# helmholtz-analytics/mpi4torch

Measured on AMD Instinct MI355X. Metric: allreduce_fwdbwd_algbw_GBps, higher is better.
Workload: dtype bf16; 1 GPU; model=allreduce_1GiB_bf16_fwd_bwd, parallelism=dp1

## Files before the change

### csrc/extension.cpp

```cpp

#include "ops.hpp"
#include "transport.hpp"

#include <torch/script.h>
#include <torch/extension.h>

#include <rccl/rccl.h>

namespace m4a {
namespace {

std::string& world_group_name() {
  static std::string name;
  return name;
}

c10::intrusive_ptr<Communicator> comm_world() {
  return c10::make_intrusive<Communicator>(world_group_name());
}

c10::intrusive_ptr<Communicator> comm_from_group(std::string group_name) {
  return c10::make_intrusive<Communicator>(std::move(group_name));
}

// ... 54 lines not shown

  m.def("_set_world_group_name",
        [](const std::string& name) { m4a::world_group_name() = name; });
  m.def("_get_world_group_name",
        []() { return m4a::world_group_name(); });

  m.def("force_host_staging",
        [](bool enabled) { m4a::config().force_host_staging = enabled; });
  m.def("host_staging_forced",
        []() { return m4a::config().force_host_staging; });

  m.def("force_full_path",
        [](bool enabled) { m4a::config().force_full_path = enabled; });

  m.def("_pack_roundtrip", &m4a::debug_pack_roundtrip);
  m.def("_slab_copy", &m4a::debug_slab_copy);
  m.def("_unpack_blocks", &m4a::debug_unpack_blocks);
  m.def("_pack_blocks", &m4a::debug_pack_blocks);
  m.def("_bitwise_reduce", &m4a::debug_bitwise_reduce);
  m.def("_fp8_reduce", &m4a::debug_fp8_reduce);
  m.def("_arith_reduce", &m4a::debug_arith_reduce);
  m.def("_pairloc_reduce", &m4a::debug_pairloc_reduce);
  m.def("_mx8_quantize", &m4a::debug_mx8_quantize);
  m.def("_mx8_reduce", &m4a::debug_mx8_reduce);
  m.def("_mx8_dequantize", &m4a::debug_mx8_dequantize, py::arg("payload"),
        py::arg("scales"), py::arg("numel"), py::arg("dtype"),
        py::arg("out") = c10::optional<at::Tensor>());
  m.def("_mx8_reduce_to", &m4a::debug_mx8_reduce_to, py::arg("payload"),
        py::arg("scales"), py::arg("numel"), py::arg("dtype"),
        py::arg("out") = c10::optional<at::Tensor>());
  m.def("_mx8_dequantize_blocks", &m4a::debug_mx8_dequantize_blocks,
// ... 30 lines not shown
```

### csrc/kernels.hip

```cpp

#include <hip/hip_runtime.h>
#include <hip/hip_fp8.h>
#include "kernels.hpp"

namespace m4a {

namespace {

struct SlabArgs {
  const char* src;
  char* dst;
  long long row_b;
  long long chunks_per_row;
  long long total_chunks;
  long long src_pitch_b;
  long long dst_pitch_b;
};

template <int N>
struct SlabPack {
  SlabArgs s[N];
};

typedef unsigned int v4u __attribute__((ext_vector_type(4)));
template <typename T>
struct NtVec {
  using type = T;
};
template <>
struct NtVec<uint4> {
  using type = v4u;
};

template <typename VecT, int NSLABS>
__global__ __launch_bounds__(256) void slab_copy_kernel(SlabPack<NSLABS> pack) {
  constexpr long long G = (long long)sizeof(VecT);
  const SlabArgs& a = pack.s[blockIdx.z];
  const long long stride = (long long)gridDim.x * blockDim.x;
  for (long long i = (long long)blockIdx.x * blockDim.x + threadIdx.x;
       i < a.total_chunks; i += stride) {
    const long long b = i / a.chunks_per_row;
    const long long c = i - b * a.chunks_per_row;
    const char* srow = a.src + b * a.src_pitch_b;
    char* drow = a.dst + b * a.dst_pitch_b;
    long long head =
        (G - ((long long)(uintptr_t)drow & (G - 1))) & (G - 1);
    if (head > a.row_b) head = a.row_b;
    const long long body = (a.row_b - head) / G;
    if (c < body) {
      using NT = typename NtVec<VecT>::type;
      const NT* sp = reinterpret_cast<const NT*>(srow + head) + c;
      NT* dp = reinterpret_cast<NT*>(drow + head) + c;
      __builtin_nontemporal_store(__builtin_nontemporal_load(sp), dp);
    } else {
      for (long long k = 0; k < head; ++k) drow[k] = srow[k];
      for (long long k = head + body * G; k < a.row_b; ++k) drow[k] = srow[k];
    }
  }
}

template <typename VecT>
void launch_bucket(const SlabDesc* descs, int n, hipStream_t stream) {
  constexpr long long G = (long long)sizeof(VecT);
  while (n > 0) {
    const int take = n < kMaxSlabsPerLaunch ? n : kMaxSlabsPerLaunch;
    SlabPack<kMaxSlabsPerLaunch> pack{};
    long long max_chunks = 0;
    for (int i = 0; i < take; ++i) {
      const SlabDesc& d = descs[i];
      SlabArgs& a = pack.s[i];
      a.src = static_cast<const char*>(d.src);
      a.dst = static_cast<char*>(d.dst);
      a.row_b = d.count * d.after_b;
      a.src_pitch_b = d.src_pitch_b;
      a.dst_pitch_b = d.dst_pitch_b;
      a.chunks_per_row = (a.row_b >= G ? a.row_b / G : 0) + 1;
      a.total_chunks = d.before * a.chunks_per_row;
      if (a.total_chunks > max_chunks) max_chunks = a.total_chunks;
    }
    for (int i = take; i < kMaxSlabsPerLaunch; ++i) {
      pack.s[i] = pack.s[0];
      pack.s[i].total_chunks = 0;
    }
    if (max_chunks > 0) {
      long long blocks = (max_chunks + 255) / 256;
      if (blocks > 4096) blocks = 4096;
      if (blocks < 1) blocks = 1;
      dim3 grid((unsigned)blocks, 1, (unsigned)take);
      hipLaunchKernelGGL((slab_copy_kernel<VecT, kMaxSlabsPerLaunch>), grid,
                         dim3(256), 0, stream, pack);
    }
    descs += take;
    n -= take;
  }
}


template <int Q>
__device__ inline uint4 byte_window_q(const unsigned int d[8], int rbits) {
  if (rbits == 0) return make_uint4(d[Q], d[Q + 1], d[Q + 2], d[Q + 3]);
  auto take = [&](int j) {
    unsigned long long w =
        ((unsigned long long)d[Q + j + 1] << 32) | d[Q + j];
    return (unsigned int)(w >> rbits);
  };
  return make_uint4(take(0), take(1), take(2), take(3));
}

__device__ inline uint4 byte_window(const uint4& lo, const uint4& hi, int s) {
  const unsigned int d[8] = {lo.x, lo.y, lo.z, lo.w, hi.x, hi.y, hi.z, hi.w};
  const int q = s >> 2;
  const int rbits = (s & 3) * 8;
  switch (q) {
    case 0: return byte_window_q<0>(d, rbits);
    case 1: return byte_window_q<1>(d, rbits);
    case 2: return byte_window_q<2>(d, rbits);
    default: return byte_window_q<3>(d, rbits);
  }
}

template <int NSLABS>
__global__ __launch_bounds__(256) void slab_copy_shift_kernel(
    SlabPack<NSLABS> pack) {
  const SlabArgs& a = pack.s[blockIdx.z];
  const long long stride = (long long)gridDim.x * blockDim.x;
  for (long long i = (long long)blockIdx.x * blockDim.x + threadIdx.x;
       i < a.total_chunks; i += stride) {
    const long long b = i / a.chunks_per_row;
    const long long c = i - b * a.chunks_per_row;
    const char* srow = a.src + b * a.src_pitch_b;
    char* drow = a.dst + b * a.dst_pitch_b;
    long long head = (16 - ((long long)(uintptr_t)drow & 15)) & 15;
    if (head > a.row_b) head = a.row_b;
    const long long body = (a.row_b - head) / 16;
    const char* sbase = srow + head;
    const int s = (int)((uintptr_t)sbase & 15);
    const long long bodyv = (s == 0) ? body : (body > 0 ? body - 1 : 0);
    const long long vs = (s == 0 || s <= head) ? 0 : 1;
    if (c >= vs && c < bodyv) {
      const char* sal = sbase - s + 16 * c;
      if (s == 0) {
        __builtin_nontemporal_store(
            __builtin_nontemporal_load(reinterpret_cast<const v4u*>(sal)),
            reinterpret_cast<v4u*>(drow + head + 16 * c));
      } else {
        const uint4 lo = *reinterpret_cast<const uint4*>(sal);
        const uint4 hi = *reinterpret_cast<const uint4*>(sal + 16);
        const uint4 w = byte_window(lo, hi, s);
        __builtin_nontemporal_store(
            *reinterpret_cast<const v4u*>(&w),
            reinterpret_cast<v4u*>(drow + head + 16 * c));
      }
    } else if (c == bodyv) {
      if (bodyv <= vs) {
        for (long long k = 0; k < a.row_b; ++k) drow[k] = srow[k];
      } else {
        const long long lo_end = head + vs * 16;
        for (long long k = 0; k < lo_end; ++k) drow[k] = srow[k];
        for (long long k = head + bodyv * 16; k < a.row_b; ++k) {
          drow[k] = srow[k];
        }
      }
    }
  }
}

void launch_shift_bucket(const SlabDesc* descs, int n, hipStream_t stream) {
  while (n > 0) {
    const int take = n < kMaxSlabsPerLaunch ? n : kMaxSlabsPerLaunch;
    SlabPack<kMaxSlabsPerLaunch> pack{};
    long long max_chunks = 0;
    for (int i = 0; i < take; ++i) {
      const SlabDesc& d = descs[i];
      SlabArgs& a = pack.s[i];
      a.src = static_cast<const char*>(d.src);
      a.dst = static_cast<char*>(d.dst);
      a.row_b = d.count * d.after_b;
      a.src_pitch_b = d.src_pitch_b;
      a.dst_pitch_b = d.dst_pitch_b;
      a.chunks_per_row = (a.row_b >= 16 ? a.row_b / 16 : 0) + 1;
      a.total_chunks = d.before * a.chunks_per_row;
      if (a.total_chunks > max_chunks) max_chunks = a.total_chunks;
    }
    for (int i = take; i < kMaxSlabsPerLaunch; ++i) {
      pack.s[i] = pack.s[0];
      pack.s[i].total_chunks = 0;
    }
    if (max_chunks > 0) {
      long long blocks = (max_chunks + 255) / 256;
      if (blocks > 4096) blocks = 4096;
      if (blocks < 1) blocks = 1;
      dim3 grid((unsigned)blocks, 1, (unsigned)take);
      hipLaunchKernelGGL((slab_copy_shift_kernel<kMaxSlabsPerLaunch>), grid,
                         dim3(256), 0, stream, pack);
    }
    descs += take;
    n -= take;
  }
}

inline int slab_granule(const SlabDesc& d) {
  const long long delta =
      (long long)((uintptr_t)d.src - (uintptr_t)d.dst);
  const long long pdelta = d.src_pitch_b - d.dst_pitch_b;
  for (int g = 16; g > 1; g >>= 1) {
    if ((delta & (g - 1)) == 0 && (pdelta & (g - 1)) == 0) return g;
  }
  return 1;
}
// ... 45 lines not shown

template <typename T, typename Op>
void launch_bitred(const void* in, void* out, int64_t chunk_elems, int nranks,
                   hipStream_t stream) {
  long long blocks = (chunk_elems + 255) / 256;
  if (blocks > 4096) blocks = 4096;
  if (blocks < 1) blocks = 1;
  hipLaunchKernelGGL((bitwise_reduce_kernel<T, Op>), dim3((unsigned)blocks),
                     dim3(256), 0, stream, static_cast<const T*>(in),
                     static_cast<T*>(out), (long long)chunk_elems,
                     (long long)nranks);
}

}

void launch_slab_copy(const SlabDesc* descs, int n, hipStream_t stream) {
  int i = 0;
  while (i < n) {
    const int g = slab_granule(descs[i]);
    int j = i + 1;
    while (j < n && slab_granule(descs[j]) == g) ++j;
    switch (g) {
      case 16: launch_bucket<uint4>(descs + i, j - i, stream); break;
      case 8: launch_bucket<unsigned long long>(descs + i, j - i, stream); break;
      case 4: launch_bucket<unsigned int>(descs + i, j - i, stream); break;
      default:
        launch_shift_bucket(descs + i, j - i, stream);
        break;
    }
    i = j;
  }
}

void launch_bitwise_reduce(const void* in, void* out, int64_t chunk_bytes,
                           int nranks, int op, hipStream_t stream) {
  const bool vec16 = (chunk_bytes % 16 == 0) &&
                     (reinterpret_cast<uintptr_t>(in) % 16 == 0) &&
                     (reinterpret_cast<uintptr_t>(out) % 16 == 0);
  if (vec16) {
    const int64_t elems = chunk_bytes / 16;
    switch (op) {
      case 0: launch_bitred<uint4, OpAnd>(in, out, elems, nranks, stream); break;
// ... 147 lines not shown
      launch_fp8_reduce_t<Op, true>(in, out, n_elems, nranks, stream);
    } else {
      launch_fp8_reduce_t<Op, false>(in, out, n_elems, nranks, stream);
    }
  };
  switch (op) {
    case 0: dispatch(FAdd{}); break;
    case 1: dispatch(FMul{}); break;
    case 2: dispatch(FMinNan{}); break;
    default: dispatch(FMaxNan{}); break;
  }
}


namespace {

constexpr long long kMaxGrid = 1ll << 30;

struct TF32 {
  using S = float;
  static constexpr int E = 4;
  __device__ static void unpack(v4u w, float* f) {
    for (int d = 0; d < 4; ++d) f[d] = __uint_as_float(w[d]);
  }
  __device__ static v4u pack(const float* f) {
    v4u o;
    for (int d = 0; d < 4; ++d) o[d] = __float_as_uint(f[d]);
    return o;
  }
  __device__ static float ld(const S* p) { return *p; }
  __device__ static void st(S* p, float f) { *p = f; }
};
// ... 122 lines not shown
    const char* __restrict__ src, char* __restrict__ dst, long long nvec,
    long long nbytes) {
  const long long items = nvec + (nbytes > nvec * 16 ? 1 : 0);
  for (long long t = blockIdx.x; t * 256 < items; t += gridDim.x) {
    const long long i = t * 256 + threadIdx.x;
    if (i < nvec) {
      __builtin_nontemporal_store(
          __builtin_nontemporal_load(reinterpret_cast<const v4u*>(src) + i),
          reinterpret_cast<v4u*>(dst) + i);
    } else if (i == nvec) {
      for (long long k = nvec * 16; k < nbytes; ++k) dst[k] = src[k];
    }
  }
}

inline unsigned arith_grid(long long items) {
  long long blocks = (items + 255) / 256;
  if (blocks > kMaxGrid) blocks = kMaxGrid;
  if (blocks < 1) blocks = 1;
  return (unsigned)blocks;
}

template <typename T, typename Op>
void launch_arith_reduce_t(const void* own, const void* staged,
                           int64_t stride_elems, int nranks, int me,
                           void* out, int64_t n, hipStream_t stream) {
  const long long esize = (long long)sizeof(typename T::S);
  const long long stride_b = (long long)stride_elems * esize;
  auto al16 = [](const void* p) {
    return reinterpret_cast<uintptr_t>(p) % 16 == 0;
  };
  const bool vec = al16(own) && al16(out) && al16(staged) && stride_b % 16 == 0;
  if (vec) {
    const long long nvec = n / T::E;
    const long long items = nvec + (n % T::E ? 1 : 0);
    hipLaunchKernelGGL((arith_reduce_kernel<T, Op>), dim3(arith_grid(items)),
                       dim3(256), 0, stream, static_cast<const char*>(own),
                       static_cast<const char*>(staged), stride_b, nranks, me,
                       static_cast<char*>(out), nvec, (long long)n);
  } else {
    hipLaunchKernelGGL((arith_reduce_kernel_scalar<T, Op>),
                       dim3(arith_grid(n)), dim3(256), 0, stream,
                       static_cast<const char*>(own),
                       static_cast<const char*>(staged), stride_b, nranks, me,
                       static_cast<char*>(out), (long long)n);
  }
}

}

void launch_arith_copy(const void* src, void* dst, int64_t nbytes,
                       hipStream_t stream) {
  if (nbytes <= 0) return;
  if (reinterpret_cast<uintptr_t>(src) % 16 != 0 ||
      reinterpret_cast<uintptr_t>(dst) % 16 != 0) {
    SlabDesc d;
    d.src = src;
    d.dst = dst;
    d.before = 1;
    d.count = 1;
    d.after_b = nbytes;
    d.src_pitch_b = nbytes;
    d.dst_pitch_b = nbytes;
    launch_slab_copy(&d, 1, stream);
    return;
  }
  const long long nvec = nbytes / 16;
  const long long items = nvec + (nbytes % 16 ? 1 : 0);
  hipLaunchKernelGGL(arith_reduce_copy_kernel, dim3(arith_grid(items)),
                     dim3(256), 0, stream, static_cast<const char*>(src),
                     static_cast<char*>(dst), nvec, (long long)nbytes);
}

void launch_arith_reduce(const void* own, const void* staged,
                         int64_t stride_elems, int nranks, int me, void* out,
                         int64_t n_elems, int op, int dtype,
                         hipStream_t stream) {
  if (n_elems <= 0) return;
  if (nranks == 1) {
    launch_arith_copy(own, out, n_elems * (dtype == 0 ? 4 : 2), stream);
    return;
  }
  auto dispatch = [&](auto opv) {
    using Op = decltype(opv);
    switch (dtype) {
      case 0:
// ... 124 lines not shown
```

### csrc/kernels.hpp

```cpp
#pragma once

#include <hip/hip_runtime_api.h>
#include <cstdint>

namespace m4a {

struct SlabDesc {
  const void* src;
  void* dst;
  int64_t before;
  int64_t count;
  int64_t after_b;
  int64_t src_pitch_b;
  int64_t dst_pitch_b;
};

constexpr int kMaxSlabsPerLaunch = 8;

void launch_slab_copy(const SlabDesc* descs, int n, hipStream_t stream);

void launch_bitwise_reduce(const void* in, void* out, int64_t chunk_bytes,
                           int nranks, int op, hipStream_t stream);

void launch_pairloc_reduce(const void* in, void* out, int64_t n_pairs,
                           int nranks, int op, int dtype, hipStream_t stream);

void launch_fp8_reduce(const void* in, void* out, int64_t n_elems,
                       int nranks, int op, bool e5m2, hipStream_t stream);

void launch_arith_reduce(const void* own, const void* staged,
                         int64_t stride_elems, int nranks, int me, void* out,
                         int64_t n_elems, int op, int dtype,
                         hipStream_t stream);
void launch_arith_copy(const void* src, void* dst, int64_t nbytes,
                       hipStream_t stream);

void launch_mx8_quantize(const void* in, void* payload, void* scales,
                         int64_t n_elems, int dtype, hipStream_t stream);
void launch_mx8_reduce(const void* payload_in, const void* scales_in,
                       void* payload_out, void* scales_out, int64_t n_groups,
                       int nranks, hipStream_t stream);
void launch_mx8_dequantize(const void* payload, const void* scales, void* out,
                           int64_t n_elems, int dtype, hipStream_t stream);
void launch_mx8_reduce_to(const void* payload_in, const void* scales_in,
                          void* out, int64_t n_elems, int nranks, int dtype,
                          hipStream_t stream);
void launch_mx8_dequantize_blocks(const void* payload, const void* scales,
                                  void* out, int nblocks, int64_t rows,
                                  int64_t row_elems, int dtype,
                                  hipStream_t stream);
// ... 6 lines not shown
```

### csrc/ops.cpp

```cpp

#include "ops.hpp"
#include "transport.hpp"
#include "kernels.hpp"

#include <torch/csrc/autograd/function.h>
#include <torch/csrc/autograd/functions/utils.h>
#include <torch/csrc/autograd/variable.h>
#include <ATen/core/TensorBody.h>
#include <ATen/WrapDimUtils.h>

#include <ATen/hip/impl/HIPStreamMasqueradingAsCUDA.h>

#include <algorithm>
#include <cstdlib>
#include <cstring>
#include <functional>
#include <limits>
#include <map>
#include <mutex>
#include <tuple>

namespace m4a {

using at::Tensor;
// ... 124 lines not shown
      auto b3 = blocks[i].view({g.before, counts[i], g.after})
                    .narrow(0, row_lo, rows);
      if (pack) {
        b3.copy_(f3.narrow(1, displs[i], counts[i]));
      } else {
        f3.narrow(1, displs[i], counts[i]).copy_(b3);
      }
    }
  }
}


Tensor fast_clone(const Tensor& in) {
  if (!in.is_cuda() || in.numel() == 0) return in.clone();
  auto out = at::empty_like(in);
  SlabDesc d;
  d.src = in.data_ptr();
  d.dst = out.data_ptr();
  d.before = 1;
  d.count = 1;
  d.after_b = in.numel() * in.element_size();
  d.src_pitch_b = d.after_b;
  d.dst_pitch_b = d.after_b;
  launch_slab_copy(&d, 1, current_gpu_stream(in));
  return out;
}

std::vector<int64_t> prefix_displs(const std::vector<int64_t>& counts) {
  std::vector<int64_t> d(counts.size(), 0);
  for (size_t i = 1; i < counts.size(); ++i) d[i] = d[i - 1] + counts[i - 1];
  return d;
}

int64_t phase_count(const Tensor& t, int64_t per_rank_bytes) {
  const int64_t c = config().pipeline_chunk_bytes;
  if (c <= 0) return 1;
  if (t.is_cuda()) {
    hipStreamCaptureStatus st = hipStreamCaptureStatusNone;
    (void)hipStreamIsCapturing(current_gpu_stream(t), &st);
// ... 2440 lines not shown
              "debug_pack_blocks expects a contiguous in [rows, P, row_elems] "
              "and flat staging [P*rows*row_elems] of the same dtype and "
              "device");
  const int64_t rows = in.size(0), P = in.size(1), re = in.size(2);
  if (in.numel() == 0) return;
  auto full = in.view({rows, P * re});
  std::vector<int64_t> counts((size_t)P, re);
  auto displs = prefix_displs(counts);
  std::vector<Tensor> blocks((size_t)P);
  for (int64_t r = 0; r < P; ++r) {
    blocks[(size_t)r] = staging.narrow(0, r * rows * re, rows * re);
  }
  move_axis_blocks(full, 1, displs, counts, blocks, true);
}

void debug_slab_copy(const Tensor& src, const Tensor& dst,
                     const std::vector<std::vector<int64_t>>& descs) {
  TORCH_CHECK(src.is_cuda() && dst.is_cuda() && src.device() == dst.device(),
              "debug_slab_copy is a GPU kernel test");
  TORCH_CHECK(src.scalar_type() == at::kByte && dst.scalar_type() == at::kByte &&
                  src.dim() == 1 && dst.dim() == 1 && src.is_contiguous() &&
                  dst.is_contiguous(),
              "debug_slab_copy expects flat contiguous uint8 tensors");
  constexpr int64_t kMaxBytes = int64_t(1) << 31;
  TORCH_CHECK(src.numel() < kMaxBytes && dst.numel() < kMaxBytes);
  const char* sbase = static_cast<const char*>(src.data_ptr());
  char* dbase = static_cast<char*>(dst.data_ptr());
  TORCH_CHECK(sbase + src.numel() <= dbase || dbase + dst.numel() <= sbase,
              "debug_slab_copy: src and dst overlap");
  auto span = [](int64_t off, int64_t before, int64_t row_b, int64_t pitch,
                 int64_t numel, size_t i, const char* side) {
    TORCH_CHECK(off >= 0 && off <= numel && before >= 0 && before <= numel &&
                    row_b >= 0 && row_b <= numel && pitch >= 0 &&
                    pitch <= numel,
                "debug_slab_copy: descriptor ", i, " out of range on ", side);
    if (before == 0 || row_b == 0) return std::make_pair(off, off);
    const int64_t end = off + (before - 1) * pitch + row_b;
    TORCH_CHECK(end <= numel, "debug_slab_copy: descriptor ", i,
                " runs past the end of ", side);
    return std::make_pair(off, end);
  };
  std::vector<SlabDesc> slabs;
  std::vector<std::pair<int64_t, int64_t>> dspans;
  slabs.reserve(descs.size());
// ... 17 lines not shown
    s.dst = dbase + t[1];
    s.before = before;
    s.count = count;
    s.after_b = after_b;
    s.src_pitch_b = t[5];
    s.dst_pitch_b = t[6];
    slabs.push_back(s);
  }
  std::sort(dspans.begin(), dspans.end());
  for (size_t i = 1; i < dspans.size(); ++i) {
    TORCH_CHECK(dspans[i - 1].second <= dspans[i].first,
                "debug_slab_copy: destination ranges overlap");
  }
  TORCH_CHECK(slabs.size() < (size_t)std::numeric_limits<int>::max());
  if (slabs.empty()) return;
  launch_slab_copy(slabs.data(), (int)slabs.size(), current_gpu_stream(src));
}

Tensor debug_fp8_reduce(const Tensor& stacked, int64_t op) {
  TORCH_CHECK(stacked.is_cuda(), "debug_fp8_reduce is a GPU kernel test");
  TORCH_CHECK(stacked.dim() >= 2);
  TORCH_CHECK(stacked.scalar_type() == at::kFloat8_e4m3fn ||
              stacked.scalar_type() == at::kFloat8_e5m2);
  auto in = stacked.contiguous();
  const int64_t n = in.size(0);
  auto out = at::empty(in.sizes().slice(1).vec(), in.options());
  launch_fp8_reduce(in.data_ptr(), out.data_ptr(), out.numel(), (int)n,
                    (int)op, in.scalar_type() == at::kFloat8_e5m2,
                    current_gpu_stream(in));
  return out;
}
// ... 222 lines not shown
```

### csrc/ops.hpp

```cpp
#pragma once

#include "common.hpp"

#include <ATen/ATen.h>
#include <torch/custom_class.h>

#include <memory>
#include <mutex>
#include <string>
#include <tuple>
#include <vector>

namespace m4a {

struct Transport;

struct Communicator : torch::CustomClassHolder {
  explicit Communicator(std::string group_name);

  int64_t GetRank();
  int64_t GetSize();

  at::Tensor Allreduce(const at::Tensor& input, int64_t op);
  at::Tensor AllreduceCompressed(const at::Tensor& input, int64_t op);
// ... 46 lines not shown

 private:
  std::string group_name_;
  std::mutex mu_;
  std::shared_ptr<Transport> cpu_tr_;
  std::shared_ptr<Transport> gpu_tr_;
  int gpu_device_ = -1;
};

at::Tensor join_dummies(const at::Tensor& loopthrough,
                        const std::vector<at::Tensor>& dummies);

at::Tensor debug_pack_roundtrip(const at::Tensor& input, int64_t axis,
                                std::vector<int64_t> counts);
void debug_slab_copy(const at::Tensor& src, const at::Tensor& dst,
                     const std::vector<std::vector<int64_t>>& descs);
at::Tensor debug_bitwise_reduce(const at::Tensor& stacked, int64_t op);
at::Tensor debug_fp8_reduce(const at::Tensor& stacked, int64_t op);
at::Tensor debug_arith_reduce(const at::Tensor& own, const at::Tensor& staged,
                              int64_t me, int64_t op);
std::tuple<at::Tensor, at::Tensor> debug_mx8_quantize(const at::Tensor& x);
std::tuple<at::Tensor, at::Tensor> debug_mx8_reduce(const at::Tensor& payload,
                                                    const at::Tensor& scales);
at::Tensor debug_mx8_dequantize(const at::Tensor& payload,
                                const at::Tensor& scales, int64_t numel,
                                at::ScalarType dtype,
                                const c10::optional<at::Tensor>& out);
at::Tensor debug_mx8_reduce_to(const at::Tensor& payload,
                               const at::Tensor& scales, int64_t numel,
                               at::ScalarType dtype,
                               const c10::optional<at::Tensor>& out);
// ... 15 lines not shown
```

### csrc/transport.cpp

```cpp

#include "transport.hpp"

#include <torch/csrc/distributed/c10d/Backend.hpp>
#include <torch/csrc/distributed/c10d/ProcessGroup.hpp>
#include <torch/csrc/distributed/c10d/GroupRegistry.hpp>
#include <torch/csrc/distributed/c10d/Types.hpp>

#include <ATen/hip/HIPContext.h>
#include <ATen/hip/impl/HIPStreamMasqueradingAsCUDA.h>
#include <ATen/hip/impl/HIPCachingAllocatorMasqueradingAsCUDA.h>
#include <ATen/hip/impl/HIPGuardImplMasqueradingAsCUDA.h>

#include <hip/hip_runtime_api.h>
#include <rccl/rccl.h>

#include <atomic>
#include <cstdlib>
#include <cstring>
#include <deque>
#include <map>
#include <mutex>
#include <unordered_map>

namespace m4a {
// ... 124 lines not shown
    return e;
  }
  void release(hipEvent_t e) {
    std::lock_guard<std::mutex> g(mu_);
    free_.push_back(e);
  }

 private:
  explicit EventPool(int dev) : dev_(dev) {}
  int dev_;
  std::mutex mu_;
  std::vector<hipEvent_t> free_;
};


struct SelfMatcher {
  struct Pending {
    uint64_t req_id;
    at::Tensor buf;
    int tag;
  };
  std::mutex mu;
  std::map<int, std::deque<Pending>> sends, recvs;

  static void check_tags(int stag, int rtag) {
    if (!config().debug_collectives) return;
    TORCH_CHECK(stag == rtag,
                "mpi4torch_amd[debug]: self send/recv matched FIFO but with "
                "different tags (send tag ", stag, ", recv tag ", rtag,
                "). Matching is FIFO per (peer, channel); tags do not "
                "reorder it — reorder your posts instead.");
  }

  static void complete_pair(const at::Tensor& src, at::Tensor& dst,
                            uint64_t sreq, uint64_t rreq) {
    dst.copy_(src, true);
    auto& tab = requests();
    std::lock_guard<std::mutex> g(tab.mu);
    for (uint64_t id : {sreq, rreq}) {
      Request* r = tab.peek(id);
      if (!r) continue;
      r->self_pending = false;
      if (src.is_cuda()) {
        r->gpu = true;
        r->device = (int)src.get_device();
        auto cur = c10::hip::getCurrentHIPStreamMasqueradingAsCUDA(r->device);
        r->event = EventPool::forDevice(r->device).acquire();
        M4A_HIP_CHECK(hipEventRecord(r->event, cur.stream()));
      }
    }
  }
// ... 144 lines not shown
      "disagrees: sender posted (tag=", m[0], ", dtype=",
      (at::ScalarType)m[1], ", numel=", m[2], ") but this rank's recv "
      "expected (tag=", r.debug_expect[0], ", dtype=",
      (at::ScalarType)r.debug_expect[1], ", numel=", r.debug_expect[2],
      "). Tags do not reorder matching; make both ranks post their "
      "transfers per peer+channel in the same order.");
}


struct LocalTransport final : Transport {
  int rank() const override { return 0; }
  int size() const override { return 1; }
  bool is_gpu() const override { return false; }

  void allreduce(const at::Tensor& in, at::Tensor& out, RedOp) override {
    out.copy_(in, true);
  }
  void broadcast(at::Tensor&, int) override {}
  void reduce(at::Tensor&, RedOp, int) override {}
  void allgather_equal(const at::Tensor& in, at::Tensor& out) override {
    out.view_as(in).copy_(in, true);
  }
  void reduce_scatter_equal(const at::Tensor& in, at::Tensor& out,
                            RedOp) override {
    out.copy_(in.view_as(out), true);
  }
  void exchange(const std::vector<at::Tensor>& sendbufs,
                const std::vector<int>& speers,
                std::vector<at::Tensor>& recvbufs,
                const std::vector<int>& rpeers) override {
    TORCH_CHECK(sendbufs.size() == recvbufs.size(),
                "local exchange requires matched self pairs");
    for (size_t i = 0; i < sendbufs.size(); ++i) {
      TORCH_CHECK(speers[i] == 0 && rpeers[i] == 0);
      recvbufs[i].view({-1}).copy_(sendbufs[i].reshape({-1}), true);
    }
  }
  uint64_t iexchange(const std::vector<at::Tensor>& sendbufs,
                     const std::vector<int>& speers,
                     std::vector<at::Tensor>& recvbufs,
                     const std::vector<int>& rpeers) override {
    exchange(sendbufs, speers, recvbufs, rpeers);
    Request r;
    r.buffers = recvbufs;
    if (!recvbufs.empty() && recvbufs[0].is_cuda()) {
      r.gpu = true;
      r.device = (int)recvbufs[0].get_device();
      auto cur = c10::hip::getCurrentHIPStreamMasqueradingAsCUDA(r.device);
      r.event = EventPool::forDevice(r.device).acquire();
      M4A_HIP_CHECK(hipEventRecord(r.event, cur.stream()));
// ... 7 lines not shown
  }
  uint64_t irecv(at::Tensor& buf, int peer, int tag, Channel ch) override {
    TORCH_CHECK(peer == 0, "world_size is 1; cannot receive from rank ", peer);
    return self_matcher().irecv(buf, tag, ch);
  }
  uint64_t ireduce_scatter(const at::Tensor& in, at::Tensor& out,
                           RedOp op) override {
    return iallreduce(in.view_as(out), out, op);
  }
  uint64_t iallgather(const at::Tensor& in, at::Tensor& out) override {
    auto v = out.view_as(in);
    return iallreduce(in, v, kSum);
  }
  uint64_t iallreduce(const at::Tensor& in, at::Tensor& out,
                      RedOp) override {
    out.copy_(in, true);
    Request r;
    r.buffer = out;
    if (out.is_cuda()) {
      r.gpu = true;
      r.device = (int)out.get_device();
      auto cur = c10::hip::getCurrentHIPStreamMasqueradingAsCUDA(r.device);
      r.event = EventPool::forDevice(r.device).acquire();
      M4A_HIP_CHECK(hipEventRecord(r.event, cur.stream()));
    }
    return requests().add(std::move(r));
  }
};


struct C10dTransport final : Transport {
// ... 282 lines not shown
    }
    for (size_t j = 0; j < recvbufs.size(); ++j) {
      if (rpeers[j] == me) {
        self_recvs.push_back(&recvbufs[j]);
        continue;
      }
      if (nbytes(recvbufs[j]) == 0) continue;
      M4A_NCCL_CHECK(ncclRecv(recvbufs[j].data_ptr(), nbytes(recvbufs[j]),
                              ncclUint8, rpeers[j], comm(Channel::Coll),
                              hop.stream()));
    }
    M4A_NCCL_CHECK(ncclGroupEnd());
    TORCH_CHECK(self_sends.size() == self_recvs.size(),
                "exchange: unmatched self blocks");
    for (size_t i = 0; i < self_sends.size(); ++i) {
      M4A_HIP_CHECK(hipMemcpyAsync(
          self_recvs[i]->data_ptr(), self_sends[i]->data_ptr(),
          nbytes(*self_sends[i]), hipMemcpyDeviceToDevice, hop.stream()));
    }
  }
  uint64_t isend(const at::Tensor& buf, int peer, int tag,
                 Channel ch) override {
    if (peer == rank_) return self_matcher().isend(buf, tag, ch);
    std::lock_guard<std::mutex> g(mu_);
    check_not_capturing("Isend");
    return defer_p2p(true, buf, peer, tag, ch);
  }
  uint64_t irecv(at::Tensor& buf, int peer, int tag, Channel ch) override {
    if (peer == rank_) return self_matcher().irecv(buf, tag, ch);
    std::lock_guard<std::mutex> g(mu_);
    check_not_capturing("Irecv");
    return defer_p2p(false, buf, peer, tag, ch);
  }
// ... 27 lines not shown
    }
    for (size_t j = 0; j < recvbufs.size(); ++j) {
      if (rpeers[j] == me) {
        self_recvs.push_back(&recvbufs[j]);
        continue;
      }
      if (nbytes(recvbufs[j]) == 0) continue;
      M4A_NCCL_CHECK(ncclRecv(recvbufs[j].data_ptr(), nbytes(recvbufs[j]),
                              ncclUint8, rpeers[j], comm(Channel::Coll),
                              stream(Channel::Coll)));
    }
    M4A_NCCL_CHECK(ncclGroupEnd());
    TORCH_CHECK(self_sends.size() == self_recvs.size(),
                "iexchange: unmatched self blocks");
    for (size_t i = 0; i < self_sends.size(); ++i) {
      M4A_HIP_CHECK(hipMemcpyAsync(
          self_recvs[i]->data_ptr(), self_sends[i]->data_ptr(),
          nbytes(*self_sends[i]), hipMemcpyDeviceToDevice,
          stream(Channel::Coll)));
    }
    uint64_t id = make_gpu_request(Channel::Coll, at::Tensor());
    {
      auto& tab = requests();
      std::lock_guard<std::mutex> tg(tab.mu);
      if (Request* rq = tab.peek(id)) rq->buffers = all;
    }
    return id;
  }
  uint64_t iallgather(const at::Tensor& in, at::Tensor& out) override {
    std::lock_guard<std::mutex> g(mu_);
    check_not_capturing("Iallgather");
    enter_side(Channel::Coll, {in, out});
    M4A_NCCL_CHECK(ncclAllGather(in.data_ptr(), out.data_ptr(), nbytes(in),
                                 ncclUint8, comm(Channel::Coll),
// ... 34 lines not shown
  uint64_t iallreduce(const at::Tensor& in, at::Tensor& out,
                      RedOp op) override {
    std::lock_guard<std::mutex> g(mu_);
    check_not_capturing("Iallreduce");
    enter_side(Channel::Coll, {in, out});
    M4A_NCCL_CHECK(ncclAllReduce(in.data_ptr(), out.data_ptr(), in.numel(),
                                 nccl_reduce_dtype(in.scalar_type()),
                                 nccl_red_op(op), comm(Channel::Coll),
                                 stream(Channel::Coll)));
    return make_gpu_request(Channel::Coll, out);
  }

 private:
  static size_t nbytes(const at::Tensor& t) {
    return (size_t)t.numel() * t.element_size();
  }
  ncclComm_t comm(Channel ch) { return comms_[(int)ch]; }
  hipStream_t stream(Channel ch) { return streams_[(int)ch].stream(); }

  static bool stream_capturing(hipStream_t s) {
    hipStreamCaptureStatus st = hipStreamCaptureStatusNone;
    (void)hipStreamIsCapturing(s, &st);
    return st != hipStreamCaptureStatusNone;
  }

  void check_not_capturing(const char* what) {
    auto cur = c10::hip::getCurrentHIPStreamMasqueradingAsCUDA(device_);
    TORCH_CHECK(!stream_capturing(cur.stream()),
                "mpi4torch_amd: ", what,
                " inside hipGraph capture is not supported (its Wait may "
// ... 256 lines not shown
```

Before: 3146 GB/s.

## Route single-rank and self copies through custom vectorized copy kernel with row-tiled grids

On the single-rank (local) transport, allreduce, allgather, reduce-scatter and exchange copies now go through a custom nontemporal 16-byte copy kernel instead of tensor copy_ or hipMemcpyAsync. The same applies to self-peer copies in the RCCL transport. The slab copy kernels gain a 2D row-tiled grid layout that avoids per-element division, and the grid cap is lifted from 4096 to a configurable maximum. The intent is to reduce copy overhead and raise bandwidth on the dp1 allreduce path, at the risk that the custom kernel is slower than the runtime's tuned memcpy.

```diff
diff --git a/csrc/extension.cpp b/csrc/extension.cpp
--- a/csrc/extension.cpp
+++ b/csrc/extension.cpp
@@ -92,7 +92,10 @@
         [](bool enabled) { m4a::config().force_full_path = enabled; });
 
   m.def("_pack_roundtrip", &m4a::debug_pack_roundtrip);
-  m.def("_slab_copy", &m4a::debug_slab_copy);
+  m.def("_slab_copy", &m4a::debug_slab_copy, py::arg("src"), py::arg("dst"),
+        py::arg("descs"), py::arg("max_grid") = c10::optional<int64_t>());
+  m.def("_copy_bytes", &m4a::debug_copy_bytes, py::arg("src"), py::arg("dst"),
+        py::arg("max_grid") = c10::optional<int64_t>());
   m.def("_unpack_blocks", &m4a::debug_unpack_blocks);
   m.def("_pack_blocks", &m4a::debug_pack_blocks);
   m.def("_bitwise_reduce", &m4a::debug_bitwise_reduce);
diff --git a/csrc/kernels.hip b/csrc/kernels.hip
--- a/csrc/kernels.hip
+++ b/csrc/kernels.hip
@@ -12,7 +12,7 @@
   char* dst;
   long long row_b;
   long long chunks_per_row;
-  long long total_chunks;
+  long long before;
   long long src_pitch_b;
   long long dst_pitch_b;
 };
@@ -32,63 +32,125 @@
   using type = v4u;
 };
 
-template <typename VecT, int NSLABS>
+template <typename VecT>
+__device__ inline void slab_copy_chunk(const SlabArgs& a, long long b,
+                                       long long c) {
+  constexpr long long G = (long long)sizeof(VecT);
+  const char* srow = a.src + b * a.src_pitch_b;
+  char* drow = a.dst + b * a.dst_pitch_b;
+  long long head = (G - ((long long)(uintptr_t)drow & (G - 1))) & (G - 1);
+  if (head > a.row_b) head = a.row_b;
+  const long long body = (a.row_b - head) / G;
+  if (c < body) {
+    using NT = typename NtVec<VecT>::type;
+    const NT* sp = reinterpret_cast<const NT*>(srow + head) + c;
+    NT* dp = reinterpret_cast<NT*>(drow + head) + c;
+    __builtin_nontemporal_store(__builtin_nontemporal_load(sp), dp);
+  } else {
+    for (long long k = 0; k < head; ++k) drow[k] = srow[k];
+    for (long long k = head + body * G; k < a.row_b; ++k) drow[k] = srow[k];
+  }
+}
+
+template <bool ROWS, typename Fn>
+__device__ inline void slab_for_each_chunk(const SlabArgs& a, Fn fn) {
+  if (ROWS) {
+    for (long long b = blockIdx.y; b < a.before; b += gridDim.y) {
+      for (long long t = blockIdx.x; t * 256 < a.chunks_per_row;
+           t += gridDim.x) {
+        const long long c = t * 256 + threadIdx.x;
+        if (c < a.chunks_per_row) fn(b, c);
+      }
+    }
+  } else {
+    const long long total = a.before * a.chunks_per_row;
+    const long long stride = (long long)gridDim.x * 256;
+    for (long long i = (long long)blockIdx.x * 256 + threadIdx.x; i < total;
+         i += stride) {
+      const long long b = i / a.chunks_per_row;
+      fn(b, i - b * a.chunks_per_row);
+    }
+  }
+}
+
+template <typename VecT, int NSLABS, bool ROWS>
 __global__ __launch_bounds__(256) void slab_copy_kernel(SlabPack<NSLABS> pack) {
-  constexpr long long G = (long long)sizeof(VecT);
   const SlabArgs& a = pack.s[blockIdx.z];
-  const long long stride = (long long)gridDim.x * blockDim.x;
-  for (long long i = (long long)blockIdx.x * blockDim.x + threadIdx.x;
-       i < a.total_chunks; i += stride) {
-    const long long b = i / a.chunks_per_row;
-    const long long c = i - b * a.chunks_per_row;
-    const char* srow = a.src + b * a.src_pitch_b;
-    char* drow = a.dst + b * a.dst_pitch_b;
-    long long head =
-        (G - ((long long)(uintptr_t)drow & (G - 1))) & (G - 1);
-    if (head > a.row_b) head = a.row_b;
-    const long long body = (a.row_b - head) / G;
-    if (c < body) {
-      using NT = typename NtVec<VecT>::type;
-      const NT* sp = reinterpret_cast<const NT*>(srow + head) + c;
-      NT* dp = reinterpret_cast<NT*>(drow + head) + c;
-      __builtin_nontemporal_store(__builtin_nontemporal_load(sp), dp);
-    } else {
-      for (long long k = 0; k < head; ++k) drow[k] = srow[k];
-      for (long long k = head + body * G; k < a.row_b; ++k) drow[k] = srow[k];
-    }
-  }
+  slab_for_each_chunk<ROWS>(
+      a, [&](long long b, long long c) { slab_copy_chunk<VecT>(a, b, c); });
+}
+
+inline unsigned tile_grid(long long items, long long max_grid) {
+  if (max_grid > kMaxGrid) max_grid = kMaxGrid;
+  if (max_grid < 1) max_grid = 1;
+  long long blocks = (items + 255) / 256;
+  if (blocks > max_grid) blocks = max_grid;
+  if (blocks < 1) blocks = 1;
+  return (unsigned)blocks;
+}
+
+constexpr long long kRowLayoutMinTiles = 4;
+
+constexpr size_t kTileGridMinGranule = 16;
+constexpr long long kLegacyMaxGrid = 4096;
+
+bool slab_layout(const SlabDesc* descs, int take, long long G, bool tiled,
+                 long long max_grid, SlabPack<kMaxSlabsPerLaunch>& pack,
+                 dim3& grid, bool& rows) {
+  long long max_chunks = 0, max_cpr = 0, max_before = 0;
+  rows = tiled;
+  if (max_grid < 1) max_grid = 1;
+  if (!tiled && max_grid > kLegacyMaxGrid) max_grid = kLegacyMaxGrid;
+  for (int i = 0; i < take; ++i) {
+    const SlabDesc& d = descs[i];
+    SlabArgs& a = pack.s[i];
+    a.src = static_cast<const char*>(d.src);
+    a.dst = static_cast<char*>(d.dst);
+    a.row_b = d.count * d.after_b;
+    a.before = d.before;
+    a.src_pitch_b = d.src_pitch_b;
+    a.dst_pitch_b = d.dst_pitch_b;
+    a.chunks_per_row = (a.row_b >= G ? a.row_b / G : 0) + 1;
+    if (a.before <= 0) continue;
+    const long long chunks = a.before * a.chunks_per_row;
+    if (chunks > max_chunks) max_chunks = chunks;
+    if (a.chunks_per_row > max_cpr) max_cpr = a.chunks_per_row;
+    if (a.before > max_before) max_before = a.before;
+    if (a.chunks_per_row < kRowLayoutMinTiles * 256) rows = false;
+  }
+  for (int i = take; i < kMaxSlabsPerLaunch; ++i) {
+    pack.s[i] = pack.s[0];
+    pack.s[i].before = 0;
+  }
+  if (max_chunks <= 0) return false;
+  if (rows) {
+    long long gy = max_before < 65535 ? max_before : 65535;
+    if (gy > max_grid) gy = max_grid;
+    grid = dim3(tile_grid(max_cpr, max_grid), (unsigned)gy, (unsigned)take);
+  } else {
+    grid = dim3(tile_grid(max_chunks, max_grid), 1, (unsigned)take);
+  }
+  return true;
 }
 
 template <typename VecT>
-void launch_bucket(const SlabDesc* descs, int n, hipStream_t stream) {
-  constexpr long long G = (long long)sizeof(VecT);
+void launch_bucket(const SlabDesc* descs, int n, hipStream_t stream,
+                   long long max_grid) {
   while (n > 0) {
     const int take = n < kMaxSlabsPerLaunch ? n : kMaxSlabsPerLaunch;
     SlabPack<kMaxSlabsPerLaunch> pack{};
-    long long max_chunks = 0;
-    for (int i = 0; i < take; ++i) {
-      const SlabDesc& d = descs[i];
-      SlabArgs& a = pack.s[i];
-      a.src = static_cast<const char*>(d.src);
-      a.dst = static_cast<char*>(d.dst);
-      a.row_b = d.count * d.after_b;
-      a.src_pitch_b = d.src_pitch_b;
-      a.dst_pitch_b = d.dst_pitch_b;
-      a.chunks_per_row = (a.row_b >= G ? a.row_b / G : 0) + 1;
-      a.total_chunks = d.before * a.chunks_per_row;
-      if (a.total_chunks > max_chunks) max_chunks = a.total_chunks;
-    }
-    for (int i = take; i < kMaxSlabsPerLaunch; ++i) {
-      pack.s[i] = pack.s[0];
-      pack.s[i].total_chunks = 0;
-    }
-    if (max_chunks > 0) {
-      long long blocks = (max_chunks + 255) / 256;
-      if (blocks > 4096) blocks = 4096;
-      if (blocks < 1) blocks = 1;
-      dim3 grid((unsigned)blocks, 1, (unsigned)take);
-      hipLaunchKernelGGL((slab_copy_kernel<VecT, kMaxSlabsPerLaunch>), grid,
-                         dim3(256), 0, stream, pack);
+    dim3 grid;
+    bool rows;
+    if (slab_layout(descs, take, (long long)sizeof(VecT),
+                    sizeof(VecT) >= kTileGridMinGranule, max_grid, pack, grid,
+                    rows)) {
+      if (rows) {
+        hipLaunchKernelGGL((slab_copy_kernel<VecT, kMaxSlabsPerLaunch, true>),
+                           grid, dim3(256), 0, stream, pack);
+      } else {
+        hipLaunchKernelGGL((slab_copy_kernel<VecT, kMaxSlabsPerLaunch, false>),
+                           grid, dim3(256), 0, stream, pack);
+      }
     }
     descs += take;
     n -= take;
@@ -119,80 +181,68 @@
   }
 }
 
-template <int NSLABS>
+__device__ inline void slab_shift_chunk(const SlabArgs& a, long long b,
+                                        long long c) {
+  const char* srow = a.src + b * a.src_pitch_b;
+  char* drow = a.dst + b * a.dst_pitch_b;
+  long long head = (16 - ((long long)(uintptr_t)drow & 15)) & 15;
+  if (head > a.row_b) head = a.row_b;
+  const long long body = (a.row_b - head) / 16;
+  const char* sbase = srow + head;
+  const int s = (int)((uintptr_t)sbase & 15);
+  const long long bodyv = (s == 0) ? body : (body > 0 ? body - 1 : 0);
+  const long long vs = (s == 0 || s <= head) ? 0 : 1;
+  if (c >= vs && c < bodyv) {
+    const char* sal = sbase - s + 16 * c;
+    if (s == 0) {
+      __builtin_nontemporal_store(
+          __builtin_nontemporal_load(reinterpret_cast<const v4u*>(sal)),
+          reinterpret_cast<v4u*>(drow + head + 16 * c));
+    } else {
+      const uint4 lo = *reinterpret_cast<const uint4*>(sal);
+      const uint4 hi = *reinterpret_cast<const uint4*>(sal + 16);
+      const uint4 w = byte_window(lo, hi, s);
+      __builtin_nontemporal_store(
+          *reinterpret_cast<const v4u*>(&w),
+          reinterpret_cast<v4u*>(drow + head + 16 * c));
+    }
+  } else if (c == bodyv) {
+    if (bodyv <= vs) {
+      for (long long k = 0; k < a.row_b; ++k) drow[k] = srow[k];
+    } else {
+      const long long lo_end = head + vs * 16;
+      for (long long k = 0; k < lo_end; ++k) drow[k] = srow[k];
+      for (long long k = head + bodyv * 16; k < a.row_b; ++k) {
+        drow[k] = srow[k];
+      }
+    }
+  }
+}
+
+template <int NSLABS, bool ROWS>
 __global__ __launch_bounds__(256) void slab_copy_shift_kernel(
     SlabPack<NSLABS> pack) {
   const SlabArgs& a = pack.s[blockIdx.z];
-  const long long stride = (long long)gridDim.x * blockDim.x;
-  for (long long i = (long long)blockIdx.x * blockDim.x + threadIdx.x;
-       i < a.total_chunks; i += stride) {
-    const long long b = i / a.chunks_per_row;
-    const long long c = i - b * a.chunks_per_row;
-    const char* srow = a.src + b * a.src_pitch_b;
-    char* drow = a.dst + b * a.dst_pitch_b;
-    long long head = (16 - ((long long)(uintptr_t)drow & 15)) & 15;
-    if (head > a.row_b) head = a.row_b;
-    const long long body = (a.row_b - head) / 16;
-    const char* sbase = srow + head;
-    const int s = (int)((uintptr_t)sbase & 15);
-    const long long bodyv = (s == 0) ? body : (body > 0 ? body - 1 : 0);
-    const long long vs = (s == 0 || s <= head) ? 0 : 1;
-    if (c >= vs && c < bodyv) {
-      const char* sal = sbase - s + 16 * c;
-      if (s == 0) {
-        __builtin_nontemporal_store(
-            __builtin_nontemporal_load(reinterpret_cast<const v4u*>(sal)),
-            reinterpret_cast<v4u*>(drow + head + 16 * c));
-      } else {
-        const uint4 lo = *reinterpret_cast<const uint4*>(sal);
-        const uint4 hi = *reinterpret_cast<const uint4*>(sal + 16);
-        const uint4 w = byte_window(lo, hi, s);
-        __builtin_nontemporal_store(
-            *reinterpret_cast<const v4u*>(&w),
-            reinterpret_cast<v4u*>(drow + head + 16 * c));
-      }
-    } else if (c == bodyv) {
-      if (bodyv <= vs) {
-        for (long long k = 0; k < a.row_b; ++k) drow[k] = srow[k];
-      } else {
-        const long long lo_end = head + vs * 16;
-        for (long long k = 0; k < lo_end; ++k) drow[k] = srow[k];
-        for (long long k = head + bodyv * 16; k < a.row_b; ++k) {
-          drow[k] = srow[k];
-        }
-      }
-    }
-  }
-}
-
-void launch_shift_bucket(const SlabDesc* descs, int n, hipStream_t stream) {
+  slab_for_each_chunk<ROWS>(
+      a, [&](long long b, long long c) { slab_shift_chunk(a, b, c); });
+}
+
+void launch_shift_bucket(const SlabDesc* descs, int n, hipStream_t stream,
+                         long long max_grid) {
   while (n > 0) {
     const int take = n < kMaxSlabsPerLaunch ? n : kMaxSlabsPerLaunch;
     SlabPack<kMaxSlabsPerLaunch> pack{};
-    long long max_chunks = 0;
-    for (int i = 0; i < take; ++i) {
-      const SlabDesc& d = descs[i];
-      SlabArgs& a = pack.s[i];
-      a.src = static_cast<const char*>(d.src);
-      a.dst = static_cast<char*>(d.dst);
-      a.row_b = d.count * d.after_b;
-      a.src_pitch_b = d.src_pitch_b;
-      a.dst_pitch_b = d.dst_pitch_b;
-      a.chunks_per_row = (a.row_b >= 16 ? a.row_b / 16 : 0) + 1;
-      a.total_chunks = d.before * a.chunks_per_row;
-      if (a.total_chunks > max_chunks) max_chunks = a.total_chunks;
-    }
-    for (int i = take; i < kMaxSlabsPerLaunch; ++i) {
-      pack.s[i] = pack.s[0];
-      pack.s[i].total_chunks = 0;
-    }
-    if (max_chunks > 0) {
-      long long blocks = (max_chunks + 255) / 256;
-      if (blocks > 4096) blocks = 4096;
-      if (blocks < 1) blocks = 1;
-      dim3 grid((unsigned)blocks, 1, (unsigned)take);
-      hipLaunchKernelGGL((slab_copy_shift_kernel<kMaxSlabsPerLaunch>), grid,
-                         dim3(256), 0, stream, pack);
+    dim3 grid;
+    bool rows;
+    if (slab_layout(descs, take, 16, true, max_grid, pack, grid,
+                    rows)) {
+      if (rows) {
+        hipLaunchKernelGGL((slab_copy_shift_kernel<kMaxSlabsPerLaunch, true>),
+                           grid, dim3(256), 0, stream, pack);
+      } else {
+        hipLaunchKernelGGL((slab_copy_shift_kernel<kMaxSlabsPerLaunch, false>),
+                           grid, dim3(256), 0, stream, pack);
+      }
     }
     descs += take;
     n -= take;
@@ -268,18 +318,23 @@
 
 }
 
-void launch_slab_copy(const SlabDesc* descs, int n, hipStream_t stream) {
+void launch_slab_copy(const SlabDesc* descs, int n, hipStream_t stream,
+                      int64_t max_grid) {
   int i = 0;
   while (i < n) {
     const int g = slab_granule(descs[i]);
     int j = i + 1;
     while (j < n && slab_granule(descs[j]) == g) ++j;
     switch (g) {
-      case 16: launch_bucket<uint4>(descs + i, j - i, stream); break;
-      case 8: launch_bucket<unsigned long long>(descs + i, j - i, stream); break;
-      case 4: launch_bucket<unsigned int>(descs + i, j - i, stream); break;
+      case 16: launch_bucket<uint4>(descs + i, j - i, stream, max_grid); break;
+      case 8:
+        launch_bucket<unsigned long long>(descs + i, j - i, stream, max_grid);
+        break;
+      case 4:
+        launch_bucket<unsigned int>(descs + i, j - i, stream, max_grid);
+        break;
       default:
-        launch_shift_bucket(descs + i, j - i, stream);
+        launch_shift_bucket(descs + i, j - i, stream, max_grid);
         break;
     }
     i = j;
@@ -457,8 +512,6 @@
 
 
 namespace {
-
-constexpr long long kMaxGrid = 1ll << 30;
 
 struct TF32 {
   using S = float;
@@ -611,13 +664,6 @@
   }
 }
 
-inline unsigned arith_grid(long long items) {
-  long long blocks = (items + 255) / 256;
-  if (blocks > kMaxGrid) blocks = kMaxGrid;
-  if (blocks < 1) blocks = 1;
-  return (unsigned)blocks;
-}
-
 template <typename T, typename Op>
 void launch_arith_reduce_t(const void* own, const void* staged,
                            int64_t stride_elems, int nranks, int me,
@@ -631,13 +677,14 @@
   if (vec) {
     const long long nvec = n / T::E;
     const long long items = nvec + (n % T::E ? 1 : 0);
-    hipLaunchKernelGGL((arith_reduce_kernel<T, Op>), dim3(arith_grid(items)),
-                       dim3(256), 0, stream, static_cast<const char*>(own),
+    hipLaunchKernelGGL((arith_reduce_kernel<T, Op>),
+                       dim3(tile_grid(items, kMaxGrid)), dim3(256), 0, stream,
+                       static_cast<const char*>(own),
                        static_cast<const char*>(staged), stride_b, nranks, me,
                        static_cast<char*>(out), nvec, (long long)n);
   } else {
     hipLaunchKernelGGL((arith_reduce_kernel_scalar<T, Op>),
-                       dim3(arith_grid(n)), dim3(256), 0, stream,
+                       dim3(tile_grid(n, kMaxGrid)), dim3(256), 0, stream,
                        static_cast<const char*>(own),
                        static_cast<const char*>(staged), stride_b, nranks, me,
                        static_cast<char*>(out), (long long)n);
@@ -647,7 +694,7 @@
 }
 
 void launch_arith_copy(const void* src, void* dst, int64_t nbytes,
-                       hipStream_t stream) {
+                       hipStream_t stream, int64_t max_grid) {
   if (nbytes <= 0) return;
   if (reinterpret_cast<uintptr_t>(src) % 16 != 0 ||
       reinterpret_cast<uintptr_t>(dst) % 16 != 0) {
@@ -659,14 +706,15 @@
     d.after_b = nbytes;
     d.src_pitch_b = nbytes;
     d.dst_pitch_b = nbytes;
-    launch_slab_copy(&d, 1, stream);
+    launch_slab_copy(&d, 1, stream, max_grid);
     return;
   }
   const long long nvec = nbytes / 16;
   const long long items = nvec + (nbytes % 16 ? 1 : 0);
-  hipLaunchKernelGGL(arith_reduce_copy_kernel, dim3(arith_grid(items)),
-                     dim3(256), 0, stream, static_cast<const char*>(src),
-                     static_cast<char*>(dst), nvec, (long long)nbytes);
+  hipLaunchKernelGGL(arith_reduce_copy_kernel,
+                     dim3(tile_grid(items, max_grid)), dim3(256), 0, stream,
+                     static_cast<const char*>(src), static_cast<char*>(dst),
+                     nvec, (long long)nbytes);
 }
 
 void launch_arith_reduce(const void* own, const void* staged,
diff --git a/csrc/kernels.hpp b/csrc/kernels.hpp
--- a/csrc/kernels.hpp
+++ b/csrc/kernels.hpp
@@ -17,7 +17,10 @@
 
 constexpr int kMaxSlabsPerLaunch = 8;
 
-void launch_slab_copy(const SlabDesc* descs, int n, hipStream_t stream);
+constexpr int64_t kMaxGrid = ((int64_t(1) << 32) - 1) / 256;
+
+void launch_slab_copy(const SlabDesc* descs, int n, hipStream_t stream,
+                      int64_t max_grid = kMaxGrid);
 
 void launch_bitwise_reduce(const void* in, void* out, int64_t chunk_bytes,
                            int nranks, int op, hipStream_t stream);
@@ -33,7 +36,7 @@
                          int64_t n_elems, int op, int dtype,
                          hipStream_t stream);
 void launch_arith_copy(const void* src, void* dst, int64_t nbytes,
-                       hipStream_t stream);
+                       hipStream_t stream, int64_t max_grid = kMaxGrid);
 
 void launch_mx8_quantize(const void* in, void* payload, void* scales,
                          int64_t n_elems, int dtype, hipStream_t stream);
diff --git a/csrc/ops.cpp b/csrc/ops.cpp
--- a/csrc/ops.cpp
+++ b/csrc/ops.cpp
@@ -162,15 +162,9 @@
 Tensor fast_clone(const Tensor& in) {
   if (!in.is_cuda() || in.numel() == 0) return in.clone();
   auto out = at::empty_like(in);
-  SlabDesc d;
-  d.src = in.data_ptr();
-  d.dst = out.data_ptr();
-  d.before = 1;
-  d.count = 1;
-  d.after_b = in.numel() * in.element_size();
-  d.src_pitch_b = d.after_b;
-  d.dst_pitch_b = d.after_b;
-  launch_slab_copy(&d, 1, current_gpu_stream(in));
+  launch_arith_copy(in.data_ptr(), out.data_ptr(),
+                    in.numel() * (int64_t)in.element_size(),
+                    current_gpu_stream(in));
   return out;
 }
 
@@ -2641,20 +2635,39 @@
   move_axis_blocks(full, 1, displs, counts, blocks, true);
 }
 
-void debug_slab_copy(const Tensor& src, const Tensor& dst,
-                     const std::vector<std::vector<int64_t>>& descs) {
+namespace {
+
+constexpr int64_t kDebugCopyMaxBytes = int64_t(1) << 31;
+
+int64_t debug_copy_check(const Tensor& src, const Tensor& dst,
+                         c10::optional<int64_t> max_grid, const char* who) {
   TORCH_CHECK(src.is_cuda() && dst.is_cuda() && src.device() == dst.device(),
-              "debug_slab_copy is a GPU kernel test");
+              who, " is a GPU kernel test");
   TORCH_CHECK(src.scalar_type() == at::kByte && dst.scalar_type() == at::kByte &&
                   src.dim() == 1 && dst.dim() == 1 && src.is_contiguous() &&
                   dst.is_contiguous(),
-              "debug_slab_copy expects flat contiguous uint8 tensors");
-  constexpr int64_t kMaxBytes = int64_t(1) << 31;
-  TORCH_CHECK(src.numel() < kMaxBytes && dst.numel() < kMaxBytes);
+              who, " expects flat contiguous uint8 tensors");
+  TORCH_CHECK(src.numel() < kDebugCopyMaxBytes &&
+              dst.numel() < kDebugCopyMaxBytes);
+  const char* sbase = static_cast<const char*>(src.data_ptr());
+  const char* dbase = static_cast<const char*>(dst.data_ptr());
+  TORCH_CHECK(sbase + src.numel() <= dbase || dbase + dst.numel() <= sbase,
+              who, ": src and dst overlap");
+  const int64_t cap = max_grid.value_or(kMaxGrid);
+  TORCH_CHECK(cap >= 1 && cap <= kMaxGrid, who, ": max_grid must be in [1, ",
+              kMaxGrid, "]");
+  return cap;
+}
+
+}
+
+void debug_slab_copy(const Tensor& src, const Tensor& dst,
+                     const std::vector<std::vector<int64_t>>& descs,
+                     c10::optional<int64_t> max_grid) {
+  const int64_t cap = debug_copy_check(src, dst, max_grid, "debug_slab_copy");
+  constexpr int64_t kMaxBytes = kDebugCopyMaxBytes;
   const char* sbase = static_cast<const char*>(src.data_ptr());
   char* dbase = static_cast<char*>(dst.data_ptr());
-  TORCH_CHECK(sbase + src.numel() <= dbase || dbase + dst.numel() <= sbase,
-              "debug_slab_copy: src and dst overlap");
   auto span = [](int64_t off, int64_t before, int64_t row_b, int64_t pitch,
                  int64_t numel, size_t i, const char* side) {
     TORCH_CHECK(off >= 0 && off <= numel && before >= 0 && before <= numel &&
@@ -2702,7 +2715,17 @@
   }
   TORCH_CHECK(slabs.size() < (size_t)std::numeric_limits<int>::max());
   if (slabs.empty()) return;
-  launch_slab_copy(slabs.data(), (int)slabs.size(), current_gpu_stream(src));
+  launch_slab_copy(slabs.data(), (int)slabs.size(), current_gpu_stream(src),
+                   cap);
+}
+
+void debug_copy_bytes(const Tensor& src, const Tensor& dst,
+                      c10::optional<int64_t> max_grid) {
+  const int64_t cap = debug_copy_check(src, dst, max_grid, "debug_copy_bytes");
+  TORCH_CHECK(src.numel() == dst.numel(),
+              "debug_copy_bytes: src and dst differ in length");
+  launch_arith_copy(src.data_ptr(), dst.data_ptr(), src.numel(),
+                    current_gpu_stream(src), cap);
 }
 
 Tensor debug_fp8_reduce(const Tensor& stacked, int64_t op) {
diff --git a/csrc/ops.hpp b/csrc/ops.hpp
--- a/csrc/ops.hpp
+++ b/csrc/ops.hpp
@@ -84,7 +84,10 @@
 at::Tensor debug_pack_roundtrip(const at::Tensor& input, int64_t axis,
                                 std::vector<int64_t> counts);
 void debug_slab_copy(const at::Tensor& src, const at::Tensor& dst,
-                     const std::vector<std::vector<int64_t>>& descs);
+                     const std::vector<std::vector<int64_t>>& descs,
+                     c10::optional<int64_t> max_grid = c10::nullopt);
+void debug_copy_bytes(const at::Tensor& src, const at::Tensor& dst,
+                      c10::optional<int64_t> max_grid = c10::nullopt);
 at::Tensor debug_bitwise_reduce(const at::Tensor& stacked, int64_t op);
 at::Tensor debug_fp8_reduce(const at::Tensor& stacked, int64_t op);
 at::Tensor debug_arith_reduce(const at::Tensor& own, const at::Tensor& staged,
diff --git a/csrc/transport.cpp b/csrc/transport.cpp
--- a/csrc/transport.cpp
+++ b/csrc/transport.cpp
@@ -162,6 +162,32 @@
 };
 
 
+static bool kernel_copyable(const at::Tensor& src, const at::Tensor& dst) {
+  return src.is_cuda() && dst.is_cuda() && src.device() == dst.device() &&
+         src.is_contiguous() && dst.is_contiguous() &&
+         src.scalar_type() == dst.scalar_type() && src.numel() == dst.numel();
+}
+
+static void kernel_copy(const at::Tensor& src, const at::Tensor& dst,
+                        hipStream_t stream) {
+  c10::hip::HIPGuardMasqueradingAsCUDA guard(dst.device());
+  launch_arith_copy(src.data_ptr(), dst.data_ptr(),
+                    src.numel() * (int64_t)src.element_size(), stream);
+}
+
+static void copy_on_current_stream(const at::Tensor& src,
+                                   const at::Tensor& dst) {
+  if (kernel_copyable(src, dst)) {
+    kernel_copy(src, dst,
+                c10::hip::getCurrentHIPStreamMasqueradingAsCUDA(
+                    (int)dst.get_device())
+                    .stream());
+  } else {
+    dst.copy_(src, true);
+  }
+}
+
+
 struct SelfMatcher {
   struct Pending {
     uint64_t req_id;
@@ -182,7 +208,7 @@
 
   static void complete_pair(const at::Tensor& src, at::Tensor& dst,
                             uint64_t sreq, uint64_t rreq) {
-    dst.copy_(src, true);
+    copy_on_current_stream(src, dst);
     auto& tab = requests();
     std::lock_guard<std::mutex> g(tab.mu);
     for (uint64_t id : {sreq, rreq}) {
@@ -357,16 +383,16 @@
   bool is_gpu() const override { return false; }
 
   void allreduce(const at::Tensor& in, at::Tensor& out, RedOp) override {
-    out.copy_(in, true);
+    copy_on_current_stream(in, out);
   }
   void broadcast(at::Tensor&, int) override {}
   void reduce(at::Tensor&, RedOp, int) override {}
   void allgather_equal(const at::Tensor& in, at::Tensor& out) override {
-    out.view_as(in).copy_(in, true);
+    copy_on_current_stream(in, out.view_as(in));
   }
   void reduce_scatter_equal(const at::Tensor& in, at::Tensor& out,
                             RedOp) override {
-    out.copy_(in.view_as(out), true);
+    copy_on_current_stream(in.view_as(out), out);
   }
   void exchange(const std::vector<at::Tensor>& sendbufs,
                 const std::vector<int>& speers,
@@ -376,7 +402,11 @@
                 "local exchange requires matched self pairs");
     for (size_t i = 0; i < sendbufs.size(); ++i) {
       TORCH_CHECK(speers[i] == 0 && rpeers[i] == 0);
-      recvbufs[i].view({-1}).copy_(sendbufs[i].reshape({-1}), true);
+      if (kernel_copyable(sendbufs[i], recvbufs[i])) {
+        copy_on_current_stream(sendbufs[i], recvbufs[i]);
+      } else {
+        recvbufs[i].view({-1}).copy_(sendbufs[i].reshape({-1}), true);
+      }
     }
   }
   uint64_t iexchange(const std::vector<at::Tensor>& sendbufs,
@@ -414,7 +444,7 @@
   }
   uint64_t iallreduce(const at::Tensor& in, at::Tensor& out,
                       RedOp) override {
-    out.copy_(in, true);
+    copy_on_current_stream(in, out);
     Request r;
     r.buffer = out;
     if (out.is_cuda()) {
@@ -727,9 +757,7 @@
     TORCH_CHECK(self_sends.size() == self_recvs.size(),
                 "exchange: unmatched self blocks");
     for (size_t i = 0; i < self_sends.size(); ++i) {
-      M4A_HIP_CHECK(hipMemcpyAsync(
-          self_recvs[i]->data_ptr(), self_sends[i]->data_ptr(),
-          nbytes(*self_sends[i]), hipMemcpyDeviceToDevice, hop.stream()));
+      self_copy(*self_sends[i], *self_recvs[i], hop.stream());
     }
   }
   uint64_t isend(const at::Tensor& buf, int peer, int tag,
@@ -787,10 +815,7 @@
     TORCH_CHECK(self_sends.size() == self_recvs.size(),
                 "iexchange: unmatched self blocks");
     for (size_t i = 0; i < self_sends.size(); ++i) {
-      M4A_HIP_CHECK(hipMemcpyAsync(
-          self_recvs[i]->data_ptr(), self_sends[i]->data_ptr(),
-          nbytes(*self_sends[i]), hipMemcpyDeviceToDevice,
-          stream(Channel::Coll)));
+      self_copy(*self_sends[i], *self_recvs[i], stream(Channel::Coll));
     }
     uint64_t id = make_gpu_request(Channel::Coll, at::Tensor());
     {
@@ -855,6 +880,15 @@
  private:
   static size_t nbytes(const at::Tensor& t) {
     return (size_t)t.numel() * t.element_size();
+  }
+  static void self_copy(const at::Tensor& src, const at::Tensor& dst,
+                        hipStream_t s) {
+    if (kernel_copyable(src, dst)) {
+      kernel_copy(src, dst, s);
+    } else {
+      M4A_HIP_CHECK(hipMemcpyAsync(dst.data_ptr(), src.data_ptr(), nbytes(src),
+                                   hipMemcpyDeviceToDevice, s));
+    }
   }
   ncclComm_t comm(Channel ch) { return comms_[(int)ch]; }
   hipStream_t stream(Channel ch) { return streams_[(int)ch].stream(); }
```

Measured after the change: 3131 GB/s. No clear change (-0.5%).
